# Meryx/ComputeRayTracer

Hardware: AMD Instinct MI355X
Metric: Mrays/sec (+ HBM GB/s vs peak), 1080p 250k-tri scene, 1/2/4/8 MI355X (higher is better)
Workload: dtype f32; 1 GPU; S2 atrium250k: 253952 triangles + cornell walls/light, 1920x1080, 64 spp per step (BASELINE config 3)

## Files before the change

computeraytracer_amd/_lib.py:

```python
from __future__ import annotations

import ctypes as C
import os

_HERE = os.path.dirname(os.path.abspath(__file__))
LIB_PATH = os.environ.get("CRT_LIB") or os.path.join(_HERE, "libcrt.so")

NCOUNTERS = 8
ACCEL_NONE, ACCEL_BVH2, ACCEL_LBVH, ACCEL_PLOC = 0, 1, 2, 3
CNT = dict(rays=0, nodes=1, prims=2, paths=3, bounces=4, shadow=5, hits=6, walked=7)

_P = C.c_void_p
SIGNATURES = {
    "crt_create": (C.c_int, [C.POINTER(_P), C.c_int]),
    "crt_destroy": (None, [_P]),
    "crt_last_error": (C.c_char_p, [_P]),
    "crt_abi_version": (C.c_int, []),
    "crt_upload_scene": (C.c_int, [_P, _P, C.c_size_t, _P, C.c_size_t, _P, C.c_size_t, _P, _P]),
    "crt_set_tile": (C.c_int, [_P, C.c_uint32, C.c_uint32, C.c_uint32, C.c_uint32]),
    "crt_set_row_bands": (C.c_int, [_P, C.c_uint32, C.c_uint32, C.c_uint32]),
    "crt_build_accel": (C.c_int, [_P, C.c_int]),
    "crt_reset": (C.c_int, [_P]),
    "crt_trace": (C.c_int, [_P, C.c_uint32]),
    "crt_sync": (C.c_int, [_P]),
# ... 26 lines not shown
    "crt_gather": (C.c_int, [_P, C.c_int]),
    "crt_read_frame_rgba8": (C.c_int, [_P, _P]),
    "crt_read_frame_accum": (C.c_int, [_P, _P]),
    "crt_frame_device_buffers": (C.c_int, [_P, C.POINTER(_P), C.POINTER(_P)]),
    "crt_comm_info": (C.c_int, [_P, _P]),
    "crt_comm_destroy": (C.c_int, [_P]),
    "crt_layout_rows": (C.c_int, [C.c_uint32, C.c_uint32, C.c_uint32, C.c_uint32, _P, _P]),
    "crt_denoise": (C.c_int, [_P, _P, _P, _P]),
    "crt_read_gbuffer": (C.c_int, [_P, _P]),
    "crt_read_motion": (C.c_int, [_P, _P]),
    "crt_debug_intersect": (C.c_int, [_P, _P, C.c_size_t, _P]),
    "crt_debug_trace_rays": (C.c_int, [_P, _P, C.c_size_t, _P, _P]),
    "crt_debug_read_accel": (C.c_int, [_P, C.c_int, _P, C.c_size_t, _P]),
    "crt_debug_probes": (C.c_int, [_P, _P]),
    "crt_debug_gen_culled": (C.c_int, [_P, _P]),
    "crt_debug_math": (C.c_int, [_P, C.c_int, _P, _P, _P, C.c_size_t]),
    "crt_set_camera": (C.c_int, [_P, _P]),
    "crt_update_primitives": (C.c_int, [_P, C.c_uint32, C.c_uint32, _P]),
    "crt_transform_primitives": (C.c_int, [_P, _P, C.c_uint32]),
    "crt_read_primitives": (C.c_int, [_P, C.c_uint32, C.c_uint32, _P]),
    "crt_update_lights": (C.c_int, [_P, C.c_uint32, C.c_uint32, _P]),
    "crt_refit_accel": (C.c_int, [_P, _P]),
    "crt_debug_hit_pad": (C.c_int, [_P, _P]),
    "crt_trace_adaptive": (C.c_int, [_P, _P, _P]),
    "crt_read_adaptive": (C.c_int, [_P, _P, _P]),
    "crt_adaptive_defaults": (C.c_int, [_P]),
    "crt_denoise_adaptive": (C.c_int, [_P, _P, _P, _P, _P]),
    "crt_denoise_adaptive_defaults": (C.c_int, [_P]),
    "crt_set_sample_offset": (C.c_int, [_P, C.c_uint32]),
    "crt_sample_offset": (C.c_int, [_P, _P]),
# ... 87 lines not shown
```

computeraytracer_amd/csrc/crt_api.cpp:

```cpp
#include "crt_ctx.h"

using namespace crt;

extern "C" void crt_comm_on_destroy(crt_ctx *c);
extern "C" int crt_internal_comm_partitioned(crt_ctx *c);

namespace crt {

long long g_fail_alloc_in = 0;

namespace {
std::string g_create_error;
}

int fail(crt_ctx *c, int code, const char *fmt, ...)
{
    char buf[2048];
    va_list ap;
    va_start(ap, fmt);
    vsnprintf(buf, sizeof buf, fmt, ap);
    va_end(ap);
    if (c) c->err = buf; else g_create_error = buf;
    return code;
}
// ... 206 lines not shown
    c->s_prims = prims_scale(c->prims);
    S.hit_pad = pad_of(c->s_prims, c->camera);
    c->accel_stale = false;
    c->rf_ready = false;
    S.nf_last[0] = S.nf_last[1] = kNoHit;
    for (size_t i = c->prims.size(); i-- > 0 && S.nf_last[1] == kNoHit;)
        if (c->prims[i].category != 2u) (S.nf_last[0] == kNoHit ? S.nf_last[0] : S.nf_last[1]) = (uint32_t)i;
    camera_frame(c->camera, S.cam);

    HIPCHK(c, c->d_raw.alloc(std::max<size_t>(nprim * 80, 16)));
    if (nprim) HIPCHK(c, hipMemcpy(c->d_raw.p, primitives, nprim * 80, hipMemcpyHostToDevice));
    HIPCHK(c, c->d_spectra.alloc(nspectra * kNLambda));
    HIPCHK(c, hipMemcpy(c->d_spectra.p, spectra, nspectra * kNLambda * sizeof(float), hipMemcpyHostToDevice));
    HIPCHK(c, c->d_cie.alloc(3 * kNCie));
    HIPCHK(c, hipMemcpy(c->d_cie.p, cie, 3 * kNCie * sizeof(float), hipMemcpyHostToDevice));
    std::vector<float4> hl(nlight * 3);
    for (size_t i = 0; i < nlight; i++) light_rows(c->lights[i], &hl[3 * i]);
    HIPCHK(c, c->d_lights.alloc(hl.size()));
    HIPCHK(c, hipMemcpy(c->d_lights.p, hl.data(), hl.size() * sizeof(float4), hipMemcpyHostToDevice));
    S.spectra = c->d_spectra.p; S.cie = c->d_cie.p; S.lights = c->d_lights.p;

    c->x0 = 0; c->y0 = 0; c->tw = c->W; c->th = c->H;
    c->band = 0x40000000u; c->stride = 1; c->phase = 0;
    c->accum_bound = nullptr; c->rgba_bound = nullptr;
    c->have_scene = true;
    int rc = alloc_tile(c);
    if (rc == CRT_OK) rc = zero_state(c);
    if (rc) c->have_scene = false;
    return rc;
}
// ... 496 lines not shown
        if (value != 0 && value != 1) return fail(c, CRT_EINVAL, "crt_set_option: temporal_motion is 0 or 1");
        if (!value && (c->dn.cur.snap || c->dn.prev.snap)) c->dn.drop();
        if (!value) c->dn.snap.release();
        c->dn.motion = value != 0;
        return CRT_OK;
    }
    if (!std::strcmp(name, "frame_ring")) {
        c->frame_ring = (uint32_t)std::min<int64_t>(256, std::max<int64_t>(0, value));
        c->ring_from = c->sample + 1u;
        if (c->have_scene) { HIPCHK(c, hipSetDevice(c->device)); HIPCHK(c, hipStreamSynchronize(c->stream)); return alloc_frames(c); }
        return CRT_OK;
    }
    if (!std::strcmp(name, "wf_gen_blocks")) { c->wf_gen_blocks = (int)std::min<int64_t>(4096, std::max<int64_t>(1, value)); return CRT_OK; }
    if (!std::strcmp(name, "wf_trace_form")) { c->wf_trace_form = value == 1 ? 1 : 2; return CRT_OK; }
    if (!std::strcmp(name, "wf_cull_miss")) { c->wf_cull_miss = value != 0; return CRT_OK; }
    if (!std::strcmp(name, "wf_pipes")) { c->wf_pipes = (int)std::min<int64_t>(crt_ctx::kMaxPipes, std::max<int64_t>(1, value)); return CRT_OK; }
    if (!std::strcmp(name, "wf_pool")) { c->wf_pool = (uint32_t)std::max<int64_t>(0, value); return CRT_OK; }
    if (!std::strcmp(name, "wf_waves_per_cu")) { c->wf_waves_per_cu = (uint32_t)std::min<int64_t>(32, std::max<int64_t>(0, value)); return CRT_OK; }
    if (!std::strcmp(name, "time_kernels")) {
        c->time_kernels = value != 0; c->last_trace_kernel_launches = 0;
        HIPCHK(c, hipSetDevice(c->device));
        while (value > 1 && c->kev.size() < 2 * (size_t)std::min<int64_t>(value, 1 << 20)) {
            Event e;
            HIPCHK(c, e.create());
            c->kev.push_back(std::move(e));
        }
        return CRT_OK;
    }
    return fail(c, CRT_EINVAL, "crt_set_option: unknown option '%s'", name);
}
// ... 3 lines not shown
```

computeraytracer_amd/csrc/crt_ctx.h:

```cpp
#pragma once
#include <hip/hip_runtime.h>

#include <algorithm>
#include <cfloat>
#include <cmath>
#include <cstdarg>
#include <cstdio>
#include <cstdlib>
#include <cstring>
#include <memory>
#include <string>
#include <utility>
#include <vector>

#include "../../include/crt.h"
#include "crt_bvh.h"
#include "crt_device.h"
#include "crt_launch.h"
#include "crt_math.h"
#include "crt_wf_policy.h"

namespace crt {

struct HostPrim {
    uint32_t category;
    f3 d1, d2, d3;
    uint32_t emission, reflectance, material, index;
};

extern long long g_fail_alloc_in;

template <typename T>
struct DevBuf {
    T *p = nullptr;
// ... 121 lines not shown
    DevBuf<unsigned long long> d_counters;
    bool counting = false;
    float last_ms = 0.0f;
    uint32_t last_launches = 0;
    bool last_timed = false;
    uint32_t spp_per_launch = 0;

    int pipeline = 1;
    uint32_t wf_pool = 0;
    uint32_t wf_waves_per_cu = 0;
    int num_cu = 0;
    DevBuf<float4> w_ray_o, w_ray_d, w_sh_d, w_beta, w_radiance, w_nee, w_staging[crt::kWfRing], w_recA, w_recB;
    DevBuf<uint4> w_rng, w_misc, w_recC;
    DevBuf<float2> w_hit;
    DevBuf<uint32_t> w_vis, w_dead, w_tea;
    static constexpr int kMaxPipes = crt::kWfMaxPipes;
    int wf_pipes = 2;
    int wf_defer = 1;
    int wf_tail_walk = 1;
    int wf_gen_blocks = 128;
    int wf_trace_form = 2;
    int wf_cull_miss = 1;
    int wf_chunk = 1;
    int wf_ahead = 3;
    int wf_ring = 32;
    int wf_pool_spp = 8;
    double wf_feed = 1.0;
    std::unique_ptr<crt::WfRun> run;
    uint32_t wf_finish_at = 32768;
    uint32_t wf_flush_at = 4096;
    uint32_t wf_side_ppw = 64, wf_flush_ppw = 4;
    DevBuf<crt::WfCtl> w_ctl[kMaxPipes];
    DevBuf<crt::WfWorkQ> w_wq;
    crt::Pinned<crt::WfStatus> h_status[kMaxPipes];
    crt::WfStatus *d_status[kMaxPipes] = {};
    crt::Event ev_status[kMaxPipes][crt::kStatusRing];
    crt::Event ev_done[kMaxPipes][crt::kStatusRing];
// ... 138 lines not shown
```

computeraytracer_amd/csrc/crt_debug.cpp:

```cpp
#include "crt_ctx.h"

using namespace crt;

extern "C" {

int crt_debug_intersect(crt_ctx *c, const float *rays, size_t n, float *out)
{
    if (!c || (!rays && n) || (!out && n)) return CRT_EINVAL;
    if (!c->have_scene || c->accel_mode < 0) return fail(c, CRT_ESTATE, "crt_debug_intersect: scene + accel required");
    if (c->accel_stale) return fail(c, CRT_ESTATE, "crt_debug_intersect: primitives were updated: call crt_refit_accel or crt_build_accel first");
    HIPCHK(c, hipSetDevice(c->device));
    DevBuf<float> din, dout;
    HIPCHK(c, din.alloc(n * 8));
    hipError_t e = dout.alloc(n * 8);
    if (e == hipSuccess) e = hipMemcpyAsync(din.p, rays, n * 8 * sizeof(float), hipMemcpyHostToDevice, c->stream);
    if (e == hipSuccess) e = launch_debug_intersect(c->sc, din.p, n, dout.p, c->accel_mode == CRT_ACCEL_NONE, c->stream);
    if (e == hipSuccess) e = hipMemcpyAsync(out, dout.p, n * 8 * sizeof(float), hipMemcpyDeviceToHost, c->stream);
    if (e == hipSuccess) e = hipStreamSynchronize(c->stream);
    if (e != hipSuccess) return fail(c, CRT_EDEVICE, "crt_debug_intersect: %s", hipGetErrorString(e));
    return CRT_OK;
}

int crt_debug_trace_rays(crt_ctx *c, const float *rays, size_t n, uint32_t *out, uint64_t report[8])
{
// ... 172 lines not shown
    return CRT_OK;
}

int crt_debug_read_moments(crt_ctx *c, float *out)
{
    if (!c || !out) return CRT_EINVAL;
    CRT_TRY(dn_begin(c, "crt_debug_read_moments", 0, nullptr, 0, "", DN_UNIFORM));
    if (!c->dn.cur.valid || c->dn.cur.frame != c->frame_id || !c->dn.cur.has_m)
        return fail(c, CRT_ESTATE, "crt_debug_read_moments: no crt_denoise_svgf in this frame yet, or a crt_denoise_temporal after it "
                                   "(the CURRENT slot carries no moments)");
    const size_t n = (size_t)c->tw * c->th;
    if (n) HIPCHK(c, hipMemcpyAsync(out, c->dn.cur.m.p, n * sizeof(float4), hipMemcpyDeviceToHost, c->stream));
    return dn_finish(c, n, nullptr, nullptr, nullptr);
}

int crt_debug_hit_pad(crt_ctx *c, float *out)
{
    if (!c || !out) return CRT_EINVAL;
    if (!c->have_scene) return fail(c, CRT_ESTATE, "crt_debug_hit_pad: no scene");
    *out = c->sc.hit_pad;
    return CRT_OK;
}

}
```

computeraytracer_amd/csrc/crt_device.h:

```cpp
#pragma once
#include <hip/hip_runtime.h>
#include <stdint.h>

namespace crt {

constexpr uint32_t kNoHit = 0xFFFFFFFFu;
constexpr int kStackDepth = 64;
constexpr uint32_t kNLambda = 301;
constexpr uint32_t kNCie = 471;
constexpr int CRT_NCOUNTERS_DEV = 16;

struct DevScene {
    const float4 *prim;
    const float4 *primD;
    const uint32_t *slot_of_index;
    const float4 *nodes;
    const float4 *nodes4;
    const uint4 *nodes4q;
    const uint4 *nodes8q;
    const float *spectra;
    const float *cie;
    const float4 *lights;
    uint32_t nprim;
    uint32_t npatch;
// ... 130 lines not shown
    uint32_t band, stride, phase;
    uint32_t tiles_x, tiles_y;
    uint32_t npix_padded;
    uint32_t list_cap;
    uint32_t tail_bound;
    uint32_t n_samples;
    float4 *accum;
    uchar4 *rgba;
    uchar4 *frames;
    uint32_t frame_ring;
    const uint32_t *tea;
    uint32_t count;
    uint32_t trace_form;
    int *stack_overflow;
    uint32_t overflow_lanes;
};

struct DnReprojParams {
    double m[9];
    double eye_prev[3];
    double W, H, x0, y0;
    const float4 *accum;
    const float4 *gbuf;
    const uint32_t *key;
    const float4 *h_prev;
    const float4 *gbuf_prev;
    const uint32_t *key_prev;
    float4 *h_cur;
    uchar4 *rgba;
    float *hist;
// ... 29 lines not shown
```

computeraytracer_amd/csrc/crt_launch.h:

```cpp
#pragma once
#include <hip/hip_runtime.h>

#include <vector>

#include "../../include/crt.h"
#include "crt_bvh.h"
#include "crt_device.h"

namespace crt {

hipError_t launch_trace(const TraceParams &P, bool count, bool brute, hipStream_t stream);
hipError_t launch_trace_adaptive(const TraceParams &P, const AsTiles &A, bool count, bool brute, hipStream_t stream);
hipError_t launch_debug_intersect(const DevScene &S, const float *rays, size_t n, float *out, int brute, hipStream_t stream);
hipError_t launch_debug_math(int fn, const float *a, const float *b, float *out, size_t n, hipStream_t stream);
hipError_t launch_assemble(const void *full, void *frame, uint32_t elem_bytes, uint32_t W, uint32_t H, uint32_t world, uint32_t rows_max,
                           uint32_t band, hipStream_t stream);

hipError_t wf_launch_init(const WfParams &P, hipStream_t s);
hipError_t wf_launch_tea(const WfParams &P, uint32_t *out, hipStream_t s);
hipError_t wf_launch_shade(const WfParams &P, uint32_t it, hipStream_t s);
hipError_t wf_launch_gen(const WfParams &P, uint32_t it, hipStream_t s, const AsTiles *A);
hipError_t wf_launch_trace(const WfParams &P, uint32_t it, uint32_t trace_blocks, hipStream_t s);
int wf_trace_kernel(const WfParams &P);
hipError_t wf_launch_finish(const WfParams &P, WfFinishSegs G, uint32_t max_paths, hipStream_t s);
hipError_t wf_launch_resolve(const WfParams &P, uint32_t last_sample, hipStream_t s);
hipError_t wf_launch_resolve_adaptive(const WfParams &P, const AsTiles &A, uint32_t call_end, hipStream_t s);

hipError_t as_launch_select(const AsParams &A, bool compact, hipStream_t s);
hipError_t as_launch_commit(uint32_t *counts, const uint32_t *active, uint32_t n_active, uint32_t samples, hipStream_t s);

hipError_t build_lbvh(const float *lo, const float *hi, uint32_t n, Bvh &out, hipStream_t stream);
hipError_t build_lbvh_device(const unsigned char *d_raw, uint32_t n, float hit_pad, float4 *d_prim, float4 *d_primD,
                             uint32_t *d_slot_of_index, float *d_nodes2, uint4 *d_nodes4q, LbvhDeviceResult &res, hipStream_t stream);
template <typename T> struct DevBuf;
// ... 37 lines not shown
```

computeraytracer_amd/csrc/crt_wavefront.hip:

```cpp
#include "crt_shade.h"
#include "crt_launch.h"
#include <algorithm>

namespace crt {

#ifndef CRT_WF_STACK
#define CRT_WF_STACK 32
#endif
#ifndef CRT_WF_REFILL
#define CRT_WF_REFILL 24
#endif
#ifndef CRT_WF_INNER_RUN
#define CRT_WF_INNER_RUN 6
#endif
#ifndef CRT_WF_BURSTS
#define CRT_WF_BURSTS 4
#endif
#ifndef CRT_WF_BVH4
#define CRT_WF_BVH4 1
#endif
#ifndef CRT_WF_LEAF_AT
#define CRT_WF_LEAF_AT 32
#endif
#ifndef CRT_WF_SPEC
#define CRT_WF_SPEC 1
#endif
#ifndef CRT_WF_PATCH_RECOMPUTE
#define CRT_WF_PATCH_RECOMPUTE 20
#endif
#ifndef CRT_WF_SHADE_BLOCK
#define CRT_WF_SHADE_BLOCK 64
#endif
#ifndef CRT_WF_SHADE_MIN_WAVES
#define CRT_WF_SHADE_MIN_WAVES 1
#endif
#ifndef CRT_WF_MIN_WAVES
#define CRT_WF_MIN_WAVES 1
#endif
constexpr int kWfStack = CRT_WF_STACK;
static_assert(kWfStack == kWfStackLds, "crt_scene.cpp sizes the overflow area from kWfStackLds");
constexpr int kNoNode = 0x7FFFFFFF;
constexpr int kTraceChunk = 128;
constexpr int kRefillAt = CRT_WF_REFILL;

__device__ __forceinline__ uint32_t lane_id() { return threadIdx.x & 63u; }

#ifndef CRT_WF_NT
#define CRT_WF_NT 1
#endif
typedef float v4f __attribute__((ext_vector_type(4)));
typedef float v2f __attribute__((ext_vector_type(2)));
typedef uint32_t v4u __attribute__((ext_vector_type(4)));
#if CRT_WF_NT
// ... 672 lines not shown
    WfShard &sh = ctl->shard[ring][my_shard];
    const uint32_t n_chunks = min(sh.n_dead, P.list_cap) / 64u;
    if (j >= n_chunks) return;
    const uint32_t mine = (n_chunks - j + P.gen_blocks - 1u) / P.gen_blocks;
    const size_t region = (size_t)my_shard * P.list_cap;
    const size_t cls_stride = (size_t)P.list_cap * kWfShards;
    if (CULL) {
        const cptr4u rq = (cptr4u)S.nodes4q + 4 * (size_t)S.root4;
        const v4u Q0 = rq[0], Q1 = rq[1], Q2 = rq[2];
        const f3 qscale = f3{S.qscale[0], S.qscale[1], S.qscale[2]}, qbase = f3{S.qbase[0], S.qbase[1], S.qbase[2]};
        const f3 eye = f3{S.cam[9], S.cam[10], S.cam[11]};
        uint32_t filled = 0;
        uint32_t slot = 0, slot_of = 0xFFFFFFFFu;
        uint32_t started = 0, started_q = 0;
        uint32_t c_rays = 0, c_cull = 0;
        bool pend = false, p_valid = false;
        uint32_t p_base = 0, p_entry = 0, p_rank = 0;
        f3 p_d = f3{0.0f, 0.0f, 0.0f};
        auto list_pending = [&]() {
            const uint32_t b0 = (uint32_t)__builtin_amdgcn_readfirstlane((int)p_base);
            if (p_valid) {
                const size_t e = (size_t)(lbuf * 4u) * cls_stride + region + b0 + p_rank;
                stnt(&P.recA[e], float4{eye.x, eye.y, eye.z, bits_f(0xFFFFFFFFu)});
                stnt(&P.recB[e], float4{p_d.x, p_d.y, p_d.z, bits_f(p_entry)});
            }
        };
        for (uint32_t round = 0; round < (uint32_t)CRT_WF_GEN_ROUNDS && filled < mine; round++) {
            GenWork G;
            const uint32_t total = gen_reserve(P, my_shard, lane, mine - filled, G);
            if (total == 0u) break;
            for (uint32_t k = 0; k < total; k++) {
                const uint32_t g = k < G.n[0] ? 0u : 1u, kk = g ? k - G.n[0] : k;
                const uint32_t sg = G.q[g];
                const uint32_t w0 = G.w[g] + 64u * kk;
                const uint32_t sample_off = w0 / P.npix_padded, pp0 = w0 % P.npix_padded;
                const uint32_t tile = pp0 >> 6;
                const uint32_t lx = (tile % P.tiles_x) * 8u + (lane & 7u), ly = (tile / P.tiles_x) * 8u + (lane >> 3);
                const bool valid = lx < P.tw && ly < P.th;
                const unsigned long long mv = __ballot(valid);
                if (slot_of != filled) { slot = ldnt(&P.dead[region + (size_t)(j + filled * P.gen_blocks) * 64u + lane]); slot_of = filled; }
                f3 d = f3{0.0f, 0.0f, 0.0f};
                uint32_t sample = 0, seed = 0, lambda = 0;
                bool nan_ray = false, miss = true;
                if (valid) {
                    const uint32_t px = P.x0 + lx;
                    const uint32_t py = P.y0 + (ly / P.band) * P.band * P.stride + P.phase * P.band + ly % P.band;
                    sample = P.seg[sg].first_sample + sample_off;
                    seed = P.tea[(size_t)ly * P.tw + lx];
                    const CamRay c = camera_ray(S, px, py, sample, seed);
                    d = c.d; lambda = c.lambda; nan_ray = c.nan_ray;
                    miss = !c.nan_ray && root_step_misses(Q0, Q1, Q2, qscale, qbase, c.eye, c.d);
                }
                if (__ballot(!miss) == 0ull) {
                    if (valid) {
                        uint32_t wl[4];
                        wavelengths_of(lambda, wl);
                        const f3 c = spectral_to_xyz(S, f4{0.0f, 0.0f, 0.0f, 0.0f}, wl);
                        stnt(&P.staging[sg][(size_t)sample_off * ((size_t)P.tw * P.th) + (size_t)ly * P.tw + lx], float4{c.x, c.y, c.z, 0.0f});
                        c_cull++;
                    }
                    continue;
                }
                if (valid) {
                    const uint32_t flags = kWfAlive | kWfFresh | (lambda << kWfLambdaShift) | (sg << kWfBatchShift) | (nan_ray ? kWfNanRay : 0u);
                    stnt(&P.misc[slot], uint4{w0 + lane, flags, sample, seed});
                    c_rays++;
// ... 924 lines not shown
    A.q[pix] = qy;
    P.accum[pix] = float4{acc.x, acc.y, acc.z, a4.w};
    if (P.n_samples > 0) P.rgba[pix] = tonemap_rgba8(acc, (float)(A.base[tile] + call_end));
}

__global__ __launch_bounds__(256) void k_wf_tea(const WfParams P, uint32_t *out)
{
    const uint32_t i = blockIdx.x * 256u + threadIdx.x;
    if (i >= P.tw * P.th) return;
    const uint32_t lx = i % P.tw, ly = i / P.tw;
    const uint32_t px = P.x0 + lx;
    const uint32_t py = P.y0 + (ly / P.band) * P.band * P.stride + P.phase * P.band + ly % P.band;
    out[i] = tea(px, py * 100u);
}

__global__ void k_wf_init(const WfParams P)
{
    const uint32_t i = blockIdx.x * 256u + threadIdx.x;
    if (i < P.P && !P.keep_pool) P.misc[P.slot_base + i] = uint4{0, 0, 0, 0};
    if (i < kWfShards) {
        WfCtl *c = P.ctl;
        if (!P.keep_pool)
            for (int r = 0; r < 4; r++) {
                for (int k = 0; k < 4; k++) c->shard[r][i].n[k] = 0;
                c->shard[r][i].cur = 0; c->shard[r][i].n_dead = 0;
                for (uint32_t b = 0; b < kWfRing; b++) c->shard[r][i].alive[b] = 0;
            }
        if (i == 0) { if (P.keep_pool) c->side_count[P.batch_id] = 0; else for (uint32_t b = 0; b < kWfRing; b++) c->side_count[b] = 0; }
        if (P.reset_wq) {
            P.wq[P.batch_id].work[i].cur = 0;
// ... 8 lines not shown

hipError_t wf_launch_init(const WfParams &P, hipStream_t s)
{
    hipLaunchKernelGGL(k_wf_init, dim3(P.keep_pool ? 1u : (P.P + 255) / 256), dim3(256), 0, s, P);
    return hipGetLastError();
}

hipError_t wf_launch_tea(const WfParams &P, uint32_t *out, hipStream_t s)
{
    const size_t npix = (size_t)P.tw * P.th;
    if (npix == 0) return hipSuccess;
    hipLaunchKernelGGL(k_wf_tea, dim3((unsigned)((npix + 255) / 256)), dim3(256), 0, s, P, out);
    return hipGetLastError();
}

hipError_t wf_launch_shade(const WfParams &P, uint32_t it, hipStream_t s)
{
    const uint32_t bps = (4u * P.tail_bound + CRT_WF_SHADE_BLOCK - 1u) / CRT_WF_SHADE_BLOCK;
    const dim3 gs(P.tail_bound ? kWfShards * bps : (P.P + CRT_WF_SHADE_BLOCK - 1) / CRT_WF_SHADE_BLOCK), bs(CRT_WF_SHADE_BLOCK);
    if (P.count) hipLaunchKernelGGL((k_wf_shade<true>), gs, bs, 0, s, P, it);
    else hipLaunchKernelGGL((k_wf_shade<false>), gs, bs, 0, s, P, it);
    return hipGetLastError();
}

bool wf_gen_culls(const WfParams &P)
{
    const int k = wf_trace_kernel(P);
    return P.cull_miss != 0u && (k == 1 || k == 3) && P.sc.nprim > 4u && P.sc.root4 >= 0 && P.sc.root4 != kNoNode;
}

// ... 75 lines not shown
```

computeraytracer_amd/csrc/crt_wf_driver.cpp:

```cpp
#include <chrono>
#include <thread>

#include "crt_ctx.h"

using namespace crt;

namespace crt {


WfOptions wf_options(const crt_ctx *c)
{
    WfOptions o;
    o.tw = c->tw; o.th = c->th;
    o.wf_pool = c->wf_pool; o.wf_waves_per_cu = c->wf_waves_per_cu; o.spp_per_launch = c->spp_per_launch;
    o.wf_pool_spp = c->wf_pool_spp; o.wf_ring = c->wf_ring; o.wf_pipes = c->wf_pipes; o.wf_trace_form = c->wf_trace_form;
    o.wf_cohort = c->wf_cohort; o.wf_chunk = c->wf_chunk; o.wf_tail_walk = c->wf_tail_walk; o.wf_gen_blocks = c->wf_gen_blocks;
    o.wf_finish_at = c->wf_finish_at; o.wf_flush_at = c->wf_flush_at; o.wf_feed = c->wf_feed;
    o.quant4_tree = c->bvh4q.ok && !c->bvh8q.ok;
    return o;
}

int wf_ensure_overflow(crt_ctx *c)
{
    if (c->num_cu == 0) {
// ... 13 lines not shown
    CRT_ENSURE(c, c->w_recB, list_elems);
    CRT_ENSURE(c, c->w_recC, list_elems);
    CRT_ENSURE(c, c->w_ray_o, P);
    CRT_ENSURE(c, c->w_ray_d, P);
    CRT_ENSURE(c, c->w_sh_d, P);
    CRT_ENSURE(c, c->w_beta, P);
    CRT_ENSURE(c, c->w_radiance, P);
    CRT_ENSURE(c, c->w_nee, P);
    CRT_ENSURE(c, c->w_rng, P);
    CRT_ENSURE(c, c->w_misc, P);
    CRT_ENSURE(c, c->w_hit, P);
    CRT_ENSURE(c, c->w_vis, P);
    for (uint32_t b = 0; b < ring; b++)
        CRT_ENSURE(c, c->w_staging[b], staging_elems);
    CRT_ENSURE(c, c->w_tea, (size_t)c->tw * c->th);
    if (!c->wf_host_ready) {
        if (!c->w_wq.p) {
            HIPCHK(c, c->w_wq.alloc(kWfRing));
            HIPCHK(c, hipMemset(c->w_wq.p, 0, kWfRing * sizeof(WfWorkQ)));
        }
        if (!c->ev_fork) HIPCHK(c, c->ev_fork.create(hipEventDisableTiming));
        if (!c->pub_stream) HIPCHK(c, c->pub_stream.create(hipStreamNonBlocking));
        for (int f = 0; f < crt_ctx::kFinishStreams; f++) {
            if (!c->fin_stream[f]) {
                int least = 0, greatest = 0;
                HIPCHK(c, hipDeviceGetStreamPriorityRange(&least, &greatest));
                HIPCHK(c, c->fin_stream[f].create(hipStreamNonBlocking, least));
            }
            if (!c->ev_fin[f]) HIPCHK(c, c->ev_fin[f].create(hipEventDisableTiming));
        }
// ... 574 lines not shown
            W.ctl = c->w_ctl[p].p; W.wq = c->w_wq.p;
            W.slot_base = side_slots + g.Pp * (uint32_t)p; W.reset_wq = (p == 0) ? 1u : 0u;
            W.P = g.Pp; W.x0 = c->x0; W.y0 = c->y0; W.tw = c->tw; W.th = c->th;
            W.band = c->band; W.stride = c->stride; W.phase = c->phase;
            W.tiles_x = g.tiles_x; W.tiles_y = g.tiles_y; W.npix_padded = g.npix_padded;
            W.list_cap = g.list_cap;
            W.seg[0] = WfSeg{work_total, work_per_shard, first_sample};
            W.seg_n = 1;
            W.n_samples = n;
            W.accum = accum_ptr(c); W.rgba = rgba_ptr(c);
            W.tea = c->w_tea.p;
            W.count = c->counting ? 1u : 0u;
            W.overflow_lanes = (uint32_t)c->num_cu * wf_waves(o) * 64u;
            W.stack_overflow = c->w_overflow.p + (size_t)p * W.overflow_lanes * wf_overflow_levels(c);
            W.trace_form = (uint32_t)c->wf_trace_form;
            if (!c->pipe_stream[p]) {
                int least = 0, greatest = 0;
                HIPCHK(c, hipDeviceGetStreamPriorityRange(&least, &greatest));
                HIPCHK(c, c->pipe_stream[p].create(hipStreamNonBlocking, greatest));
            }
            r.stream[p] = c->pipe_stream[p];
            r.pipes[p].blocks_now = r.trace_blocks;
        }
        for (int p = 0; p < r.K; p++) r.rate_its += r.pipes[p].it_confirmed;
        HIPCHK(c, wf_launch_init(r.W[0], c->stream));
        HIPCHK(c, wf_launch_tea(r.W[0], c->w_tea.p, c->stream));
        HIPCHK(c, hipEventRecord(c->ev_fork, c->stream));
        for (int p = 0; p < r.K; p++) {
            HIPCHK(c, hipStreamWaitEvent(r.stream[p], c->ev_fork, 0));
            if (p > 0) HIPCHK(c, wf_launch_init(r.W[p], r.stream[p]));
        }
        HIPCHK(c, hipStreamWaitEvent(c->pub_stream, c->ev_fork, 0));
        r.live = true;
    } else {
        CRT_TRY(wf_pump(c, true));
        WfBatch nb;
        nb.n = n; nb.last_sample = last_sample; nb.id = (r.open.back().id + 1u) % r.ring; nb.as_commit = as ? as->commit : 0u;
        const uint32_t id = nb.id;
        r.seg_total[id] = work_total; r.seg_wps[id] = work_per_shard;
        r.queue_left[id] = r.work_left = true;
        r.consumed[id] = 0;
// ... 49 lines not shown
```

computeraytracer_amd/renderer.py:

```python
from __future__ import annotations

import ctypes as C

import numpy as np

from . import _lib
from ._lib import ACCEL_BVH2, ACCEL_LBVH, ACCEL_NONE, ACCEL_PLOC, CNT, CrtError, NCOUNTERS
from .scene import PackedScene

_ACCEL = {"none": ACCEL_NONE, "brute": ACCEL_NONE, "bvh2": ACCEL_BVH2, "bvh": ACCEL_BVH2, "lbvh": ACCEL_LBVH, ACCEL_LBVH: ACCEL_LBVH,
          "ploc": ACCEL_PLOC, ACCEL_PLOC: ACCEL_PLOC, ACCEL_NONE: ACCEL_NONE, ACCEL_BVH2: ACCEL_BVH2}


class Renderer:
    def __init__(self, device: int = 0):
        self._lib = _lib.load()
        h = C.c_void_p()
        rc = self._lib.crt_create(C.byref(h), int(device))
        if rc != 0:
            raise CrtError(rc, (self._lib.crt_last_error(None) or b"").decode())
        self._h = h
        self.device = int(device)
        self.scene: PackedScene | None = None

# ... 429 lines not shown
        for what, (name, dtype, cols) in enumerate(self.ACCEL_PARTS, 1):
            a = part(what, dtype)
            out[name] = a.reshape(-1, cols) if cols > 1 else a
        return out

    def debug_probes(self) -> list:
        out = np.zeros(8, np.uint64)
        self._chk(self._lib.crt_debug_probes(self._h, out.ctypes.data))
        return [int(v) for v in out]

    def gen_culled(self) -> int:
        n = C.c_uint64()
        self._chk(self._lib.crt_debug_gen_culled(self._h, C.byref(n)))
        return int(n.value)

    def debug_math(self, fn: int, a, b=None) -> np.ndarray:
        a = np.ascontiguousarray(a, np.float32)
        b = np.ascontiguousarray(b if b is not None else np.zeros_like(a), np.float32)
        out = np.empty_like(a)
        self._chk(self._lib.crt_debug_math(self._h, int(fn), a.ctypes.data, b.ctypes.data, out.ctypes.data, a.size))
        return out
```

include/crt.h:

```cpp
#ifndef CRT_H
#define CRT_H

#include <stddef.h>
#include <stdint.h>

#ifdef __cplusplus
extern "C" {
#endif

#define CRT_ABI_VERSION 2

enum {
    CRT_OK = 0,
    CRT_EINVAL = -1,
    CRT_EDEVICE = -2,
    CRT_ESTATE = -3,
    CRT_ENOMEM = -4
};

enum {
    CRT_ACCEL_NONE = 0,
    CRT_ACCEL_BVH2 = 1,
    CRT_ACCEL_LBVH = 2,
    CRT_ACCEL_PLOC = 3
// ... 157 lines not shown
int crt_set_option(crt_ctx *ctx, const char *name, int64_t value);

int crt_accel_stats(crt_ctx *ctx, uint64_t out[8]);

int crt_debug_intersect(crt_ctx *ctx, const float *rays, size_t n, float *out);
int crt_debug_trace_rays(crt_ctx *ctx, const float *rays, size_t n, uint32_t *out, uint64_t report[8]);
int crt_debug_math(crt_ctx *ctx, int fn, const float *a, const float *b, float *out, size_t n);
enum {
    CRT_ACCEL_PART_HEADER = 0, CRT_ACCEL_PART_NODES2 = 1, CRT_ACCEL_PART_NODES4 = 2, CRT_ACCEL_PART_NODES4Q = 3,
    CRT_ACCEL_PART_NODES8Q = 4, CRT_ACCEL_PART_PRIM = 5, CRT_ACCEL_PART_PRIMD = 6, CRT_ACCEL_PART_SLOT_OF_INDEX = 7
};
#define CRT_ACCEL_HEADER_N 32
int crt_debug_read_accel(crt_ctx *ctx, int what, void *out, size_t capacity, size_t *bytes);
int crt_debug_probes(crt_ctx *ctx, uint64_t out[8]);
int crt_debug_gen_culled(crt_ctx *ctx, uint64_t *out);

#ifdef __cplusplus
}
#endif
#endif
```

Before: 7731 Mrays/s.

## Classify 8x8 tiles against the root node with interval arithmetic to cull primary rays

Adds a setup kernel that runs once per trace and uses conservative interval arithmetic over each pixel's jittered camera-ray directions to classify every 8x8 tile against the quantised 4-wide root node. Tiles whose rays all miss the root skip ray generation and get zero written to staging, when the spectral tables show that culled rays contribute nothing. Tiles whose rays all enter the root skip the per-ray root test. The goal is to cut work in the generation stage. The cost is an extra kernel launch and memset per trace call, plus a global word load per tile in gen. In a closed Cornell-style scene most tiles will be Enter or Maybe, so any gain is limited to the generation stage.

New measurement: 7845 Mrays/s (median of 6 runs). 1.5% higher.

```diff
diff --git a/computeraytracer_amd/_lib.py b/computeraytracer_amd/_lib.py
--- a/computeraytracer_amd/_lib.py
+++ b/computeraytracer_amd/_lib.py
@@ -64,6 +64,9 @@
     "crt_debug_read_accel": (C.c_int, [_P, C.c_int, _P, C.c_size_t, _P]),
     "crt_debug_probes": (C.c_int, [_P, _P]),
     "crt_debug_gen_culled": (C.c_int, [_P, _P]),
+    "crt_debug_tile_classes": (C.c_int, [_P, _P, C.c_size_t]),
+    "crt_debug_tile_classes_host": (C.c_int, [_P, _P, C.c_size_t]),
+    "crt_debug_tile_class_setups": (C.c_int, [_P, _P]),
     "crt_debug_math": (C.c_int, [_P, C.c_int, _P, _P, _P, C.c_size_t]),
     "crt_set_camera": (C.c_int, [_P, _P]),
     "crt_update_primitives": (C.c_int, [_P, C.c_uint32, C.c_uint32, _P]),
diff --git a/computeraytracer_amd/csrc/crt_api.cpp b/computeraytracer_amd/csrc/crt_api.cpp
--- a/computeraytracer_amd/csrc/crt_api.cpp
+++ b/computeraytracer_amd/csrc/crt_api.cpp
@@ -244,6 +244,7 @@
     HIPCHK(c, hipMemcpy(c->d_spectra.p, spectra, nspectra * kNLambda * sizeof(float), hipMemcpyHostToDevice));
     HIPCHK(c, c->d_cie.alloc(3 * kNCie));
     HIPCHK(c, hipMemcpy(c->d_cie.p, cie, 3 * kNCie * sizeof(float), hipMemcpyHostToDevice));
+    c->cie_zero = tc_culled_is_zero(cie);
     std::vector<float4> hl(nlight * 3);
     for (size_t i = 0; i < nlight; i++) light_rows(c->lights[i], &hl[3 * i]);
     HIPCHK(c, c->d_lights.alloc(hl.size()));
@@ -770,6 +771,7 @@
     if (!std::strcmp(name, "wf_gen_blocks")) { c->wf_gen_blocks = (int)std::min<int64_t>(4096, std::max<int64_t>(1, value)); return CRT_OK; }
     if (!std::strcmp(name, "wf_trace_form")) { c->wf_trace_form = value == 1 ? 1 : 2; return CRT_OK; }
     if (!std::strcmp(name, "wf_cull_miss")) { c->wf_cull_miss = value != 0; return CRT_OK; }
+    if (!std::strcmp(name, "wf_cull_classes")) { c->wf_cull_classes = value != 0; return CRT_OK; }
     if (!std::strcmp(name, "wf_pipes")) { c->wf_pipes = (int)std::min<int64_t>(crt_ctx::kMaxPipes, std::max<int64_t>(1, value)); return CRT_OK; }
     if (!std::strcmp(name, "wf_pool")) { c->wf_pool = (uint32_t)std::max<int64_t>(0, value); return CRT_OK; }
     if (!std::strcmp(name, "wf_waves_per_cu")) { c->wf_waves_per_cu = (uint32_t)std::min<int64_t>(32, std::max<int64_t>(0, value)); return CRT_OK; }
diff --git a/computeraytracer_amd/csrc/crt_ctx.h b/computeraytracer_amd/csrc/crt_ctx.h
--- a/computeraytracer_amd/csrc/crt_ctx.h
+++ b/computeraytracer_amd/csrc/crt_ctx.h
@@ -18,6 +18,7 @@
 #include "crt_device.h"
 #include "crt_launch.h"
 #include "crt_math.h"
+#include "crt_tile_class.h"
 #include "crt_wf_policy.h"
 
 namespace crt {
@@ -169,6 +170,7 @@
     DevBuf<uint4> w_rng, w_misc, w_recC;
     DevBuf<float2> w_hit;
     DevBuf<uint32_t> w_vis, w_dead, w_tea;
+    DevBuf<uint32_t> w_tile_cls;
     static constexpr int kMaxPipes = crt::kWfMaxPipes;
     int wf_pipes = 2;
     int wf_defer = 1;
@@ -176,6 +178,9 @@
     int wf_gen_blocks = 128;
     int wf_trace_form = 2;
     int wf_cull_miss = 1;
+    int wf_cull_classes = 1;
+    uint64_t tile_cls_setups = 0;
+    bool cie_zero = false;
     int wf_chunk = 1;
     int wf_ahead = 3;
     int wf_ring = 32;
diff --git a/computeraytracer_amd/csrc/crt_debug.cpp b/computeraytracer_amd/csrc/crt_debug.cpp
--- a/computeraytracer_amd/csrc/crt_debug.cpp
+++ b/computeraytracer_amd/csrc/crt_debug.cpp
@@ -210,6 +210,58 @@
     return dn_finish(c, n, nullptr, nullptr, nullptr);
 }
 
+static int tile_class_inputs(crt_ctx *c, const char *what, size_t n_tiles, WfParams &W)
+{
+    if (!c->have_scene || c->accel_mode < 0) return fail(c, CRT_ESTATE, "%s: scene + accel required", what);
+    if (c->accel_stale) return fail(c, CRT_ESTATE, "%s: primitives were updated: call crt_refit_accel or crt_build_accel first", what);
+    CRT_TRY(quiesce(c, true));
+    W = WfParams{};
+    W.sc = c->sc;
+    W.x0 = c->x0; W.y0 = c->y0; W.tw = c->tw; W.th = c->th; W.band = c->band; W.stride = c->stride; W.phase = c->phase;
+    W.tiles_x = (c->tw + 7u) / 8u; W.tiles_y = (c->th + 7u) / 8u;
+    if (c->accel_mode != CRT_ACCEL_BVH2 || c->pipeline != 1 || !W.sc.nodes4q || W.sc.root4 < 0 || W.sc.root4 == 0x7FFFFFFF)
+        return fail(c, CRT_ESTATE, "%s: no quantised 4-wide tree with an inner root", what);
+    if (n_tiles != (size_t)W.tiles_x * W.tiles_y) return fail(c, CRT_EINVAL, "%s: the tile rectangle has %zu tiles of 8x8, not %zu", what, (size_t)W.tiles_x * W.tiles_y, n_tiles);
+    return CRT_OK;
+}
+
+int crt_debug_tile_classes(crt_ctx *c, uint8_t *out, size_t n_tiles)
+{
+    if (!c || (!out && n_tiles)) return CRT_EINVAL;
+    WfParams W;
+    CRT_TRY(tile_class_inputs(c, "crt_debug_tile_classes", n_tiles, W));
+    if (n_tiles == 0) return CRT_OK;
+    const size_t words = (n_tiles + 15u) / 16u;
+    CRT_ENSURE(c, c->w_tile_cls, words);
+    std::vector<uint32_t> h(words);
+    HIPCHK(c, wf_launch_tile_classes(W, c->w_tile_cls.p, c->stream));
+    HIPCHK(c, hipMemcpyAsync(h.data(), c->w_tile_cls.p, words * sizeof(uint32_t), hipMemcpyDeviceToHost, c->stream));
+    HIPCHK(c, hipStreamSynchronize(c->stream));
+    for (size_t t = 0; t < n_tiles; t++) out[t] = (uint8_t)((h[t >> 4] >> (2u * (t & 15u))) & 3u);
+    return CRT_OK;
+}
+
+int crt_debug_tile_classes_host(crt_ctx *c, uint8_t *out, size_t n_tiles)
+{
+    if (!c || (!out && n_tiles)) return CRT_EINVAL;
+    WfParams W;
+    CRT_TRY(tile_class_inputs(c, "crt_debug_tile_classes_host", n_tiles, W));
+    TcRoot R;
+    HIPCHK(c, hipMemcpy(R.q, W.sc.nodes4q + 4 * (size_t)W.sc.root4, sizeof R.q, hipMemcpyDeviceToHost));
+    R.qscale = f3{W.sc.qscale[0], W.sc.qscale[1], W.sc.qscale[2]}; R.qbase = f3{W.sc.qbase[0], W.sc.qbase[1], W.sc.qbase[2]};
+    const TcCam C = tc_cam(W.sc.cam, W.sc.W, W.sc.H);
+    const TcTiles T{W.x0, W.y0, W.tw, W.th, W.band, W.stride, W.phase, W.tiles_x};
+    for (size_t t = 0; t < n_tiles; t++) out[t] = (uint8_t)tc_tile_class(C, R, T, (uint32_t)t);
+    return CRT_OK;
+}
+
+int crt_debug_tile_class_setups(crt_ctx *c, uint64_t *out)
+{
+    if (!c || !out) return CRT_EINVAL;
+    *out = c->tile_cls_setups;
+    return CRT_OK;
+}
+
 int crt_debug_hit_pad(crt_ctx *c, float *out)
 {
     if (!c || !out) return CRT_EINVAL;
diff --git a/computeraytracer_amd/csrc/crt_device.h b/computeraytracer_amd/csrc/crt_device.h
--- a/computeraytracer_amd/csrc/crt_device.h
+++ b/computeraytracer_amd/csrc/crt_device.h
@@ -168,6 +168,8 @@
     uint32_t trace_form;
     int *stack_overflow;
     uint32_t overflow_lanes;
+    const uint32_t *tile_cls;
+    uint32_t cls_miss_zero;
 };
 
 struct DnReprojParams {
diff --git a/computeraytracer_amd/csrc/crt_launch.h b/computeraytracer_amd/csrc/crt_launch.h
--- a/computeraytracer_amd/csrc/crt_launch.h
+++ b/computeraytracer_amd/csrc/crt_launch.h
@@ -18,6 +18,8 @@
 
 hipError_t wf_launch_init(const WfParams &P, hipStream_t s);
 hipError_t wf_launch_tea(const WfParams &P, uint32_t *out, hipStream_t s);
+hipError_t wf_launch_tile_classes(const WfParams &P, uint32_t *out, hipStream_t s);
+bool wf_gen_culls(const WfParams &P);
 hipError_t wf_launch_shade(const WfParams &P, uint32_t it, hipStream_t s);
 hipError_t wf_launch_gen(const WfParams &P, uint32_t it, hipStream_t s, const AsTiles *A);
 hipError_t wf_launch_trace(const WfParams &P, uint32_t it, uint32_t trace_blocks, hipStream_t s);
diff --git a/computeraytracer_amd/csrc/crt_tile_class.h b/computeraytracer_amd/csrc/crt_tile_class.h
--- /dev/null
+++ b/computeraytracer_amd/csrc/crt_tile_class.h
@@ -0,0 +1,208 @@
+#pragma once
+#include "crt_math.h"
+
+namespace crt {
+
+constexpr uint32_t kTcMaybe = 0, kTcMiss = 1, kTcEnter = 2;
+constexpr uint32_t kTcGrid = 16;
+constexpr uint32_t kTcNLambda = 301, kTcNCie = 471;
+
+struct TcCam { f3 llc, hor, ver, eye; float W, H; };
+struct TcRoot { uint32_t q[12]; f3 qscale, qbase; };
+struct TcTiles { uint32_t x0, y0, tw, th, band, stride, phase, tiles_x; };
+
+CRT_HD TcCam tc_cam(const float cam[12], uint32_t W, uint32_t H)
+{
+    return TcCam{f3{cam[0], cam[1], cam[2]}, f3{cam[3], cam[4], cam[5]}, f3{cam[6], cam[7], cam[8]}, f3{cam[9], cam[10], cam[11]},
+                 (float)W, (float)H};
+}
+
+CRT_HD bool tc_pixel(const TcTiles &T, uint32_t tile, uint32_t l, uint32_t &px, uint32_t &py)
+{
+    const uint32_t lx = (tile % T.tiles_x) * 8u + (l & 7u), ly = (tile / T.tiles_x) * 8u + (l >> 3);
+    px = T.x0 + lx;
+    py = T.y0 + (ly / T.band) * T.band * T.stride + T.phase * T.band + ly % T.band;
+    return lx < T.tw && ly < T.th;
+}
+
+CRT_HD bool tc_finite(float v) { return abs_(v) <= 3.402823466e38f; }
+
+CRT_HD float tc_film(float base, float sgrid, float j, float n) { return (base + (sgrid + j) / (float)kTcGrid) / n; }
+CRT_HD f3 tc_camera_dir(const TcCam &C, uint32_t px, uint32_t py, uint32_t sample, float jx, float jy)
+{
+    const float fs = tc_film((float)px, (float)(sample % kTcGrid), jx, C.W);
+    const float ft = tc_film(C.H - (float)py, (float)(sample % kTcGrid), jy, C.H);
+    return normalize(((C.llc + C.hor * fs) + C.ver * ft) - C.eye);
+}
+
+CRT_HD float tc_clamp(float d) { const float tiny = 1.0e-20f; return abs_(d) > tiny ? d : __builtin_copysignf(tiny, d); }
+CRT_HD float tc_plane(const TcRoot &R, uint32_t axis, bool hi, uint32_t k)
+{
+    const uint32_t w = R.q[(hi ? 6u : 0u) + 2u * axis + (k >> 1)];
+    return (float)((k & 1u) ? w >> 16 : w & 0xFFFFu);
+}
+
+CRT_HD bool tc_root_step_misses(const TcRoot &R, f3 ro, f3 rd)
+{
+    const float t_min = 0.001f, t_max = bits_f(0x7F800000u);
+    const float rdv[3] = {rd.x, rd.y, rd.z}, rov[3] = {ro.x, ro.y, ro.z};
+    const float qs[3] = {R.qscale.x, R.qscale.y, R.qscale.z}, qb[3] = {R.qbase.x, R.qbase.y, R.qbase.z};
+    float oid[3], id[3];
+    bool g[3];
+    for (int a = 0; a < 3; a++) {
+        const float i3 = 1.0f / tc_clamp(rdv[a]);
+        oid[a] = fma_(qb[a], i3, -(rov[a] * i3));
+        id[a] = qs[a] * i3;
+        g[a] = i3 < 0.0f;
+    }
+    bool miss = true;
+    for (uint32_t k = 0; k < 4u; k++) {
+        float n[3], f[3];
+        for (uint32_t a = 0; a < 3u; a++) {
+            n[a] = fma_(tc_plane(R, a, g[a], k), id[a], oid[a]);
+            f[a] = fma_(tc_plane(R, a, !g[a], k), id[a], oid[a]);
+        }
+        const float tn = __builtin_fmaxf(__builtin_fmaxf(n[0], n[1]), __builtin_fmaxf(n[2], t_min));
+        const float tf = __builtin_fminf(__builtin_fminf(f[0], f[1]), __builtin_fminf(f[2], t_max));
+        const float key = (tn <= tf * 1.0000005f) ? tn : 3.0e38f;
+        if (key < 3.0e38f) miss = false;
+    }
+    return miss;
+}
+
+struct iv { float lo, hi; };
+CRT_HD iv iv_pt(float v) { return iv{v, v}; }
+CRT_HD bool iv_finite(iv a) { return tc_finite(a.lo) && tc_finite(a.hi); }
+CRT_HD iv iv_hull(float a, float b, float c, float d)
+{
+    if (a != a || b != b || c != c || d != d) return iv{bits_f(0x7FC00000u), bits_f(0x7FC00000u)};
+    return iv{min_(min_(a, b), min_(c, d)), max_(max_(a, b), max_(c, d))};
+}
+CRT_HD iv iv_add(iv a, iv b) { return iv{a.lo + b.lo, a.hi + b.hi}; }
+CRT_HD iv iv_sub(iv a, iv b) { return iv{a.lo - b.hi, a.hi - b.lo}; }
+CRT_HD iv iv_neg(iv a) { return iv{-a.hi, -a.lo}; }
+CRT_HD iv iv_mul(iv a, iv b) { return iv_hull(a.lo * b.lo, a.lo * b.hi, a.hi * b.lo, a.hi * b.hi); }
+CRT_HD iv iv_div(iv a, iv b) { return iv_hull(a.lo / b.lo, a.lo / b.hi, a.hi / b.lo, a.hi / b.hi); }
+CRT_HD iv iv_fma(iv a, iv b, iv c)
+{
+    const iv l = iv_hull(fma_(a.lo, b.lo, c.lo), fma_(a.lo, b.hi, c.lo), fma_(a.hi, b.lo, c.lo), fma_(a.hi, b.hi, c.lo));
+    const iv h = iv_hull(fma_(a.lo, b.lo, c.hi), fma_(a.lo, b.hi, c.hi), fma_(a.hi, b.lo, c.hi), fma_(a.hi, b.hi, c.hi));
+    return iv{l.lo, h.hi};
+}
+CRT_HD iv iv_sq(iv a)
+{
+    const iv r = iv_hull(a.lo * a.lo, a.hi * a.hi, a.lo * a.lo, a.hi * a.hi);
+    return (a.lo <= 0.0f && a.hi >= 0.0f) ? iv{0.0f, r.hi} : r;
+}
+CRT_HD iv iv_fma_sq(iv a, iv c)
+{
+    const iv l = iv_hull(fma_(a.lo, a.lo, c.lo), fma_(a.hi, a.hi, c.lo), fma_(a.lo, a.lo, c.lo), fma_(a.hi, a.hi, c.lo));
+    const iv h = iv_hull(fma_(a.lo, a.lo, c.hi), fma_(a.hi, a.hi, c.hi), fma_(a.lo, a.lo, c.hi), fma_(a.hi, a.hi, c.hi));
+    return (a.lo <= 0.0f && a.hi >= 0.0f) ? iv{fma_(0.0f, 0.0f, c.lo), h.hi} : iv{l.lo, h.hi};
+}
+CRT_HD iv iv_max(iv a, iv b) { return iv{__builtin_fmaxf(a.lo, b.lo), __builtin_fmaxf(a.hi, b.hi)}; }
+CRT_HD iv iv_min(iv a, iv b) { return iv{__builtin_fminf(a.lo, b.lo), __builtin_fminf(a.hi, b.hi)}; }
+
+struct TcPart { iv oid, id; bool near_hi, ok; };
+CRT_HD TcPart tc_part(iv d, bool negative, float ro, float qscale, float qbase)
+{
+    TcPart p;
+    iv c;
+    if (negative) c = iv{tc_clamp(d.lo < 0.0f ? d.lo : -0.0f), tc_clamp(d.hi < 0.0f ? d.hi : -0.0f)};
+    else c = iv{tc_clamp(d.lo > 0.0f ? d.lo : 0.0f), tc_clamp(d.hi > 0.0f ? d.hi : 0.0f)};
+    const iv i3 = iv{1.0f / c.hi, 1.0f / c.lo};
+    p.oid = iv_fma(iv_pt(qbase), i3, iv_neg(iv_mul(iv_pt(ro), i3)));
+    p.id = iv_mul(iv_pt(qscale), i3);
+    p.near_hi = negative;
+    p.ok = iv_finite(i3) && iv_finite(p.oid) && iv_finite(p.id);
+    return p;
+}
+
+CRT_HD uint32_t tc_pixel_class(const TcCam &C, const TcRoot &R, uint32_t px, uint32_t py)
+{
+    const float t_min = 0.001f, t_max = bits_f(0x7F800000u);
+    const float jmax = bits_f(0x3F7FFFFFu);
+    const iv fs = iv{tc_film((float)px, 0.0f, 0.0f, C.W), tc_film((float)px, (float)(kTcGrid - 1u), jmax, C.W)};
+    const iv ft = iv{tc_film(C.H - (float)py, 0.0f, 0.0f, C.H), tc_film(C.H - (float)py, (float)(kTcGrid - 1u), jmax, C.H)};
+    const float llc[3] = {C.llc.x, C.llc.y, C.llc.z}, hor[3] = {C.hor.x, C.hor.y, C.hor.z}, ver[3] = {C.ver.x, C.ver.y, C.ver.z};
+    const float eye[3] = {C.eye.x, C.eye.y, C.eye.z};
+    const float qs[3] = {R.qscale.x, R.qscale.y, R.qscale.z}, qb[3] = {R.qbase.x, R.qbase.y, R.qbase.z};
+    iv v[3];
+    bool ok = iv_finite(fs) && iv_finite(ft) && tc_finite(eye[0]) && tc_finite(eye[1]) && tc_finite(eye[2]);
+    for (int a = 0; a < 3; a++) {
+        v[a] = iv_sub(iv_add(iv_add(iv_pt(llc[a]), iv_mul(iv_pt(hor[a]), fs)), iv_mul(iv_pt(ver[a]), ft)), iv_pt(eye[a]));
+        ok = ok && iv_finite(v[a]);
+    }
+    const iv len2 = iv_fma_sq(v[2], iv_fma_sq(v[1], iv_sq(v[0])));
+    const iv len = iv{sqrt_(len2.lo), sqrt_(len2.hi)};
+    ok = ok && iv_finite(len2) && iv_finite(len) && len.lo > 0.0f;
+    if (!ok) return kTcMaybe;
+    iv d[3];
+    for (int a = 0; a < 3; a++) {
+        d[a] = iv_div(v[a], len);
+        if (!iv_finite(d[a])) return kTcMaybe;
+    }
+    bool all_miss = true, all_enter = true;
+    for (uint32_t combo = 0; combo < 8u; combo++) {
+        TcPart p[3];
+        bool exists = true;
+        for (uint32_t a = 0; a < 3u; a++) {
+            const bool negative = ((combo >> a) & 1u) != 0u;
+            if (negative ? !(d[a].lo <= 0.0f) : !(d[a].hi >= 0.0f)) { exists = false; break; }
+            p[a] = tc_part(d[a], negative, eye[a], qs[a], qb[a]);
+        }
+        if (!exists) continue;
+        if (!p[0].ok || !p[1].ok || !p[2].ok) return kTcMaybe;
+        bool some_enter = false;
+        for (uint32_t k = 0; k < 4u; k++) {
+            iv n[3], f[3];
+            for (uint32_t a = 0; a < 3u; a++) {
+                n[a] = iv_fma(iv_pt(tc_plane(R, a, p[a].near_hi, k)), p[a].id, p[a].oid);
+                f[a] = iv_fma(iv_pt(tc_plane(R, a, !p[a].near_hi, k)), p[a].id, p[a].oid);
+                if (!iv_finite(n[a]) || !iv_finite(f[a])) return kTcMaybe;
+            }
+            const iv tn = iv_max(iv_max(n[0], n[1]), iv_max(n[2], iv_pt(t_min)));
+            const iv tf = iv_min(iv_min(f[0], f[1]), iv_min(f[2], iv_pt(t_max)));
+            if (!(tn.lo > tf.hi * 1.0000005f)) all_miss = false;
+            if (tn.hi <= tf.lo * 1.0000005f && tn.hi < 3.0e38f) some_enter = true;
+        }
+        if (!some_enter) all_enter = false;
+    }
+    return all_miss ? kTcMiss : all_enter ? kTcEnter : kTcMaybe;
+}
+
+CRT_HD uint32_t tc_tile_class(const TcCam &C, const TcRoot &R, const TcTiles &T, uint32_t tile)
+{
+    bool any = false, all_miss = true, all_enter = true;
+    for (uint32_t l = 0; l < 64u; l++) {
+        uint32_t px, py;
+        if (!tc_pixel(T, tile, l, px, py)) continue;
+        const uint32_t cls = tc_pixel_class(C, R, px, py);
+        any = true;
+        all_miss = all_miss && cls == kTcMiss;
+        all_enter = all_enter && cls == kTcEnter;
+    }
+    return !any ? kTcMaybe : all_miss ? kTcMiss : all_enter ? kTcEnter : kTcMaybe;
+}
+
+CRT_HD f3 tc_culled_xyz(const float *cie, uint32_t lambda0)
+{
+    const uint32_t wl[4] = {lambda0, (lambda0 + 4u) % kTcNLambda, (lambda0 + 8u) % kTcNLambda, (lambda0 + 12u) % kTcNLambda};
+    const float *X = cie, *Y = cie + kTcNCie, *Z = cie + 2 * kTcNCie;
+    const f4 zero = f4{0.0f, 0.0f, 0.0f, 0.0f};
+    const f4 xb = f4{X[wl[0] + 40], X[wl[1] + 40], X[wl[2] + 40], X[wl[3] + 40]};
+    const f4 yb = f4{Y[wl[0] + 40], Y[wl[1] + 40], Y[wl[2] + 40], Y[wl[3] + 40]};
+    const f4 zb = f4{Z[wl[0] + 40], Z[wl[1] + 40], Z[wl[2] + 40], Z[wl[3] + 40]};
+    const f3 xyzc = f3{dot(xb, zero), dot(yb, zero), dot(zb, zero)};
+    return (xyzc * 300.0f) / (106.856895f * 4.0f);
+}
+CRT_HD bool tc_culled_is_zero(const float *cie)
+{
+    for (uint32_t l = 0; l < kTcNLambda; l++) {
+        const f3 c = tc_culled_xyz(cie, l);
+        if (f_bits(c.x) != 0u || f_bits(c.y) != 0u || f_bits(c.z) != 0u) return false;
+    }
+    return true;
+}
+
+}
diff --git a/computeraytracer_amd/csrc/crt_wavefront.hip b/computeraytracer_amd/csrc/crt_wavefront.hip
--- a/computeraytracer_amd/csrc/crt_wavefront.hip
+++ b/computeraytracer_amd/csrc/crt_wavefront.hip
@@ -1,4 +1,5 @@
 #include "crt_shade.h"
+#include "crt_tile_class.h"
 #include "crt_launch.h"
 #include <algorithm>
 
@@ -37,6 +38,7 @@
 #ifndef CRT_WF_MIN_WAVES
 #define CRT_WF_MIN_WAVES 1
 #endif
+static_assert(kTcGrid == kGrid && kTcNLambda == kNLambda && kTcNCie == kNCie, "crt_tile_class.h restates these");
 constexpr int kWfStack = CRT_WF_STACK;
 static_assert(kWfStack == kWfStackLds, "crt_scene.cpp sizes the overflow area from kWfStackLds");
 constexpr int kNoNode = 0x7FFFFFFF;
@@ -739,6 +741,9 @@
         uint32_t slot = 0, slot_of = 0xFFFFFFFFu;
         uint32_t started = 0, started_q = 0;
         uint32_t c_rays = 0, c_cull = 0;
+        typedef const __attribute__((address_space(4))) uint32_t *cptr1u;
+        const cptr1u tile_cls = (cptr1u)P.tile_cls;
+        uint32_t cls_word = 0, cls_word_of = 0xFFFFFFFFu;
         bool pend = false, p_valid = false;
         uint32_t p_base = 0, p_entry = 0, p_rank = 0;
         f3 p_d = f3{0.0f, 0.0f, 0.0f};
@@ -763,6 +768,18 @@
                 const uint32_t lx = (tile % P.tiles_x) * 8u + (lane & 7u), ly = (tile / P.tiles_x) * 8u + (lane >> 3);
                 const bool valid = lx < P.tw && ly < P.th;
                 const unsigned long long mv = __ballot(valid);
+                uint32_t cls = kTcMaybe;
+                if (tile_cls) {
+                    if (cls_word_of != (tile >> 4)) { cls_word_of = tile >> 4; cls_word = tile_cls[cls_word_of]; }
+                    cls = (cls_word >> (2u * (tile & 15u))) & 3u;
+                }
+                if (cls == kTcMiss && P.cls_miss_zero) {
+                    if (valid) {
+                        stnt(&P.staging[sg][(size_t)sample_off * ((size_t)P.tw * P.th) + (size_t)ly * P.tw + lx], float4{0.0f, 0.0f, 0.0f, 0.0f});
+                        c_cull++;
+                    }
+                    continue;
+                }
                 if (slot_of != filled) { slot = ldnt(&P.dead[region + (size_t)(j + filled * P.gen_blocks) * 64u + lane]); slot_of = filled; }
                 f3 d = f3{0.0f, 0.0f, 0.0f};
                 uint32_t sample = 0, seed = 0, lambda = 0;
@@ -774,7 +791,7 @@
                     seed = P.tea[(size_t)ly * P.tw + lx];
                     const CamRay c = camera_ray(S, px, py, sample, seed);
                     d = c.d; lambda = c.lambda; nan_ray = c.nan_ray;
-                    miss = !c.nan_ray && root_step_misses(Q0, Q1, Q2, qscale, qbase, c.eye, c.d);
+                    miss = cls == kTcEnter ? false : !c.nan_ray && root_step_misses(Q0, Q1, Q2, qscale, qbase, c.eye, c.d);
                 }
                 if (__ballot(!miss) == 0ull) {
                     if (valid) {
@@ -1729,6 +1746,28 @@
     out[i] = tea(px, py * 100u);
 }
 
+__global__ __launch_bounds__(64) void k_wf_tile_classes(const WfParams P, uint32_t *out)
+{
+    const DevScene &S = P.sc;
+    const uint32_t lane = lane_id(), tile = blockIdx.x;
+    if (tile >= P.tiles_x * P.tiles_y) return;
+    const uint4 *rq = S.nodes4q + 4 * (size_t)S.root4;
+    const uint4 Q0 = rq[0], Q1 = rq[1], Q2 = rq[2];
+    TcRoot R;
+    R.q[0] = Q0.x; R.q[1] = Q0.y; R.q[2] = Q0.z; R.q[3] = Q0.w; R.q[4] = Q1.x; R.q[5] = Q1.y; R.q[6] = Q1.z; R.q[7] = Q1.w;
+    R.q[8] = Q2.x; R.q[9] = Q2.y; R.q[10] = Q2.z; R.q[11] = Q2.w;
+    R.qscale = f3{S.qscale[0], S.qscale[1], S.qscale[2]}; R.qbase = f3{S.qbase[0], S.qbase[1], S.qbase[2]};
+    const TcCam C = tc_cam(S.cam, S.W, S.H);
+    const TcTiles T{P.x0, P.y0, P.tw, P.th, P.band, P.stride, P.phase, P.tiles_x};
+    uint32_t px, py;
+    const bool valid = tc_pixel(T, tile, lane, px, py);
+    const uint32_t cls = valid ? tc_pixel_class(C, R, px, py) : kTcMaybe;
+    const unsigned long long mv = __ballot(valid);
+    const unsigned long long not_miss = __ballot(valid && cls != kTcMiss), not_enter = __ballot(valid && cls != kTcEnter);
+    const uint32_t tcls = mv == 0ull ? kTcMaybe : not_miss == 0ull ? kTcMiss : not_enter == 0ull ? kTcEnter : kTcMaybe;
+    if (lane == 0 && tcls != 0u) atomicOr(&out[tile >> 4], tcls << (2u * (tile & 15u)));
+}
+
 __global__ void k_wf_init(const WfParams P)
 {
     const uint32_t i = blockIdx.x * 256u + threadIdx.x;
@@ -1767,6 +1806,17 @@
     return hipGetLastError();
 }
 
+hipError_t wf_launch_tile_classes(const WfParams &P, uint32_t *out, hipStream_t s)
+{
+    const size_t n_tiles = (size_t)P.tiles_x * P.tiles_y;
+    if (n_tiles == 0) return hipSuccess;
+    if (!out || !P.sc.nodes4q || P.sc.root4 < 0 || P.sc.root4 == kNoNode) return hipErrorInvalidValue;
+    const hipError_t e = hipMemsetAsync(out, 0, ((n_tiles + 15) / 16) * sizeof(uint32_t), s);
+    if (e != hipSuccess) return e;
+    hipLaunchKernelGGL(k_wf_tile_classes, dim3((unsigned)n_tiles), dim3(64), 0, s, P, out);
+    return hipGetLastError();
+}
+
 hipError_t wf_launch_shade(const WfParams &P, uint32_t it, hipStream_t s)
 {
     const uint32_t bps = (4u * P.tail_bound + CRT_WF_SHADE_BLOCK - 1u) / CRT_WF_SHADE_BLOCK;
diff --git a/computeraytracer_amd/csrc/crt_wf_driver.cpp b/computeraytracer_amd/csrc/crt_wf_driver.cpp
--- a/computeraytracer_amd/csrc/crt_wf_driver.cpp
+++ b/computeraytracer_amd/csrc/crt_wf_driver.cpp
@@ -51,6 +51,7 @@
     for (uint32_t b = 0; b < ring; b++)
         CRT_ENSURE(c, c->w_staging[b], staging_elems);
     CRT_ENSURE(c, c->w_tea, (size_t)c->tw * c->th);
+    CRT_ENSURE(c, c->w_tile_cls, ((size_t)((c->tw + 7u) / 8u) * ((c->th + 7u) / 8u) + 15u) / 16u);
     if (!c->wf_host_ready) {
         if (!c->w_wq.p) {
             HIPCHK(c, c->w_wq.alloc(kWfRing));
@@ -655,6 +656,8 @@
             W.overflow_lanes = (uint32_t)c->num_cu * wf_waves(o) * 64u;
             W.stack_overflow = c->w_overflow.p + (size_t)p * W.overflow_lanes * wf_overflow_levels(c);
             W.trace_form = (uint32_t)c->wf_trace_form;
+            W.tile_cls = (!as && c->wf_cull_classes && wf_gen_culls(W)) ? c->w_tile_cls.p : nullptr;
+            W.cls_miss_zero = c->cie_zero ? 1u : 0u;
             if (!c->pipe_stream[p]) {
                 int least = 0, greatest = 0;
                 HIPCHK(c, hipDeviceGetStreamPriorityRange(&least, &greatest));
@@ -666,6 +669,7 @@
         for (int p = 0; p < r.K; p++) r.rate_its += r.pipes[p].it_confirmed;
         HIPCHK(c, wf_launch_init(r.W[0], c->stream));
         HIPCHK(c, wf_launch_tea(r.W[0], c->w_tea.p, c->stream));
+        if (r.W[0].tile_cls) { HIPCHK(c, wf_launch_tile_classes(r.W[0], c->w_tile_cls.p, c->stream)); c->tile_cls_setups++; }
         HIPCHK(c, hipEventRecord(c->ev_fork, c->stream));
         for (int p = 0; p < r.K; p++) {
             HIPCHK(c, hipStreamWaitEvent(r.stream[p], c->ev_fork, 0));
diff --git a/computeraytracer_amd/renderer.py b/computeraytracer_amd/renderer.py
--- a/computeraytracer_amd/renderer.py
+++ b/computeraytracer_amd/renderer.py
@@ -467,6 +467,20 @@
         self._chk(self._lib.crt_debug_gen_culled(self._h, C.byref(n)))
         return int(n.value)
 
+    def tile_classes(self, host: bool = False) -> np.ndarray:
+        t = np.zeros(4, np.uint32)
+        self._chk(self._lib.crt_tile(self._h, t.ctypes.data))
+        ty, tx = (int(t[3]) + 7) // 8, (int(t[2]) + 7) // 8
+        out = np.zeros((ty, tx), np.uint8)
+        fn = self._lib.crt_debug_tile_classes_host if host else self._lib.crt_debug_tile_classes
+        self._chk(fn(self._h, out.ctypes.data, out.size))
+        return out
+
+    def tile_class_setups(self) -> int:
+        n = C.c_uint64()
+        self._chk(self._lib.crt_debug_tile_class_setups(self._h, C.byref(n)))
+        return int(n.value)
+
     def debug_math(self, fn: int, a, b=None) -> np.ndarray:
         a = np.ascontiguousarray(a, np.float32)
         b = np.ascontiguousarray(b if b is not None else np.zeros_like(a), np.float32)
diff --git a/include/crt.h b/include/crt.h
--- a/include/crt.h
+++ b/include/crt.h
@@ -195,6 +195,9 @@
 int crt_debug_read_accel(crt_ctx *ctx, int what, void *out, size_t capacity, size_t *bytes);
 int crt_debug_probes(crt_ctx *ctx, uint64_t out[8]);
 int crt_debug_gen_culled(crt_ctx *ctx, uint64_t *out);
+int crt_debug_tile_classes(crt_ctx *ctx, uint8_t *out, size_t n_tiles);
+int crt_debug_tile_classes_host(crt_ctx *ctx, uint8_t *out, size_t n_tiles);
+int crt_debug_tile_class_setups(crt_ctx *ctx, uint64_t *out);
 
 #ifdef __cplusplus
 }
```
